# nianticlabs/simplerecon

Hardware: AMD Instinct MI355X
Metric: depth frames/sec (640x480, 7 src views, 64 planes) (higher is better)
Workload: dtype f32

## Files before the change

### simplerecon_amd/csrc/sr_pw_tiled.hip

```cpp
#include <stdlib.h>

#include "sr_common.h"

namespace {

typedef float pt_f16 __attribute__((ext_vector_type(16)));
typedef float pt_f4 __attribute__((ext_vector_type(4)));

constexpr int PT_KS = 32;
constexpr int PT_AROW = PT_KS + 4;

struct SrPtParams {
  const float* in; int in_sp;
  const float* wp;
  const float* bias; const float* gate;
  const float* res; int res_sp;
  float* out; int out_sp;
  int64_t part_stride;
  int M, HW, Cin, Cout, Co_pad, G;
  int slabs, slabs_per_part, ksplit, tiles_n;
  float slope;
};

template <int WM, int WN, int NTW, bool GATE>
__global__ __launch_bounds__(256, 2) void sr_pw_tiled_kernel(SrPtParams p) {
  constexpr int BM = 32 * WM, BN = 32 * WN * NTW;
  constexpr int A_FLOATS = BM * PT_AROW, B_FLOATS = (PT_KS / 8) * 2 * BN * 4;
  constexpr int A_PER_THREAD = BM * (PT_KS / 4) / 256;
  constexpr int B_PER_THREAD = (PT_KS / 8) * 2 * BN / 256;
  static_assert(WM * WN == 4 && A_PER_THREAD >= 1 && B_PER_THREAD >= 1, "4 waves; whole float4s per thread");
  extern __shared__ __attribute__((aligned(16))) float lds[];
  const int tid = threadIdx.x, lane = tid & 63, wave = __builtin_amdgcn_readfirstlane(tid >> 6);
  const int i = lane & 31, kk = lane >> 5;
  const int wm = wave / WN, wn = wave % WN;
  const int tile_n = blockIdx.x % p.tiles_n, tile_m = blockIdx.x / p.tiles_n;
  const int kpart = blockIdx.y;
  const int m0 = tile_m * BM, n0 = tile_n * BN;
  const int s_begin = kpart * p.slabs_per_part, s_end = min(p.slabs, s_begin + p.slabs_per_part);

  int a_row[A_PER_THREAD];
  const float* a_ptr[A_PER_THREAD];
  const float* g_ptr[A_PER_THREAD];
  const int a_q = tid & 7;
#pragma unroll
  for (int u = 0; u < A_PER_THREAD; ++u) {
    a_row[u] = (tid >> 3) + 32 * u;
    const int m = m0 + a_row[u];
    const bool ok = m < p.M;
    a_ptr[u] = ok ? p.in + (int64_t)m * p.in_sp + 4 * a_q : nullptr;
    g_ptr[u] = (GATE && ok) ? p.gate + (int64_t)(m / p.HW) * p.Cin + 4 * a_q : nullptr;
  }
  auto stage_load = [&](int s, pt_f4 (&ra)[A_PER_THREAD], pt_f4 (&rb)[B_PER_THREAD]) {
    const int k0 = s * PT_KS;
#pragma unroll
    for (int u = 0; u < A_PER_THREAD; ++u) {
      pt_f4 v = {0.f, 0.f, 0.f, 0.f};
      if (a_ptr[u] && k0 + 4 * a_q < p.Cin) {
        v = *reinterpret_cast<const pt_f4*>(a_ptr[u] + k0);
        if (GATE) v = v * *reinterpret_cast<const pt_f4*>(g_ptr[u] + k0);
      }
      ra[u] = v;
    }
#pragma unroll
    for (int u = 0; u < B_PER_THREAD; ++u) {
      const int e = tid + 256 * u;
      const int gh = e / BN, col = e - gh * BN;
      const int g = s * (PT_KS / 8) + (gh >> 1);
      pt_f4 v = {0.f, 0.f, 0.f, 0.f};
      if (g < p.G && n0 + col < p.Co_pad)
        v = *reinterpret_cast<const pt_f4*>(p.wp + ((int64_t)(g * 2 + (gh & 1)) * p.Co_pad + n0 + col) * 4);
      rb[u] = v;
    }
  };
  auto stage_store = [&](int buf, const pt_f4 (&ra)[A_PER_THREAD], const pt_f4 (&rb)[B_PER_THREAD]) {
    float* A = lds + buf * (A_FLOATS + B_FLOATS);
    float* Bt = A + A_FLOATS;
#pragma unroll
    for (int u = 0; u < A_PER_THREAD; ++u) *reinterpret_cast<pt_f4*>(&A[a_row[u] * PT_AROW + 4 * a_q]) = ra[u];
#pragma unroll
    for (int u = 0; u < B_PER_THREAD; ++u) *reinterpret_cast<pt_f4*>(&Bt[(tid + 256 * u) * 4]) = rb[u];
  };

  pt_f16 acc[NTW];
#pragma unroll
  for (int n = 0; n < NTW; ++n)
#pragma unroll
    for (int r = 0; r < 16; ++r) acc[n][r] = 0.0f;

  pt_f4 ra[A_PER_THREAD], rb[B_PER_THREAD];
  if (s_begin < s_end) {
    stage_load(s_begin, ra, rb);
    stage_store(0, ra, rb);
  }
  __syncthreads();
  for (int s = s_begin; s < s_end; ++s) {
    const int buf = (s - s_begin) & 1;
    const bool more = s + 1 < s_end;
    if (more) stage_load(s + 1, ra, rb);
    const float* A = lds + buf * (A_FLOATS + B_FLOATS);
    const float* Bt = A + A_FLOATS;
    const float* a_base = A + (32 * wm + i) * PT_AROW + 4 * kk;
    const float* b_base = Bt + (kk * BN + 32 * wn * NTW + i) * 4;
#pragma unroll
    for (int gl = 0; gl < PT_KS / 8; ++gl) {
      const pt_f4 a = *reinterpret_cast<const pt_f4*>(a_base + 8 * gl);
      pt_f4 b[NTW];
#pragma unroll
      for (int n = 0; n < NTW; ++n) b[n] = *reinterpret_cast<const pt_f4*>(b_base + (gl * 2 * BN + 32 * n) * 4);
#pragma unroll
      for (int e = 0; e < 4; ++e)
#pragma unroll
        for (int n = 0; n < NTW; ++n) acc[n] = __builtin_amdgcn_mfma_f32_32x32x2f32(a[e], b[n][e], acc[n], 0, 0, 0);
    }
    if (more) stage_store(buf ^ 1, ra, rb);
    __syncthreads();
  }

  const bool partial = p.ksplit > 1;
  const float slope = sr_uniform(partial ? -1.0f : p.slope);
  float* outp = p.out + (partial ? (int64_t)kpart * p.part_stride : (int64_t)0);
  const int rbase = m0 + 32 * wm + 4 * kk;
#pragma unroll
  for (int n = 0; n < NTW; ++n) {
    const int col = n0 + 32 * (wn * NTW + n) + i;
    const bool okc = col < p.Cout;
    const float bv = (!partial && p.bias && okc) ? p.bias[col] : 0.0f;
    float v[16];
#pragma unroll
    for (int r = 0; r < 16; ++r) v[r] = acc[n][r] + bv;
    if (!partial && p.res) {
      float rv[16];
#pragma unroll
      for (int r = 0; r < 16; ++r) {
        const int m = rbase + (r & 3) + 8 * (r >> 2);
        rv[r] = (okc && m < p.M) ? p.res[(int64_t)m * p.res_sp + col] : 0.0f;
      }
#pragma unroll
      for (int r = 0; r < 16; ++r) v[r] += rv[r];
    }
    sr_activate_group(v, slope);
#pragma unroll
    for (int r = 0; r < 16; ++r) {
      const int m = rbase + (r & 3) + 8 * (r >> 2);
      if (okc && m < p.M) outp[(int64_t)m * p.out_sp + col] = v[r];
    }
  }
}

int pt_num_cus() { return sr_device_cus(); }

struct PtPlan { int cfg, ks; };
constexpr int PT_BM[4] = {64, 128, 128, 64}, PT_BN[4] = {128, 160, 64, 64};

PtPlan pt_plan(int M, int Cin, int Cout, bool can_split) {
  const int f_cfg = sr_opt(SR_OPT_PT_CFG), f_ks = sr_opt(SR_OPT_PT_KS);
  const int slabs = (Cin + PT_KS - 1) / PT_KS;
  const long want = (long)pt_num_cus() * 3 / 2;
  PtPlan best = {0, 1};
  double best_cost = -1.0;
  for (int cfg = 0; cfg < 4; ++cfg) {
    if (f_cfg >= 0 && cfg != f_cfg) continue;
    const long tm = (M + PT_BM[cfg] - 1) / PT_BM[cfg], tn = (Cout + PT_BN[cfg] - 1) / PT_BN[cfg];
    const double pad = (double)(tm * PT_BM[cfg]) * (double)(tn * PT_BN[cfg]) / ((double)M * Cout);
    for (int ks = 1; ks <= 8; ks *= 2) {
      if (f_ks > 0 && ks != f_ks) continue;
      if (ks > 1 && (!can_split || slabs / ks < 4)) continue;
      const long wgs = tm * tn * ks;
      const double fill = wgs >= want ? 1.0 : (double)want / (double)wgs;
      const double reuse = 1.0 + 24.0 / (PT_BM[cfg] * PT_BN[cfg] / (double)(PT_BM[cfg] + PT_BN[cfg]));
      const double cost = pad * fill * reuse * (1.0 + (ks > 1 ? 0.10 + 2.0 * ks / slabs : 0.0));
      if (best_cost < 0 || cost < best_cost) { best = {cfg, ks}; best_cost = cost; }
    }
  }
  return best;
}

template <int WM, int WN, int NTW>
int pt_launch(const SrPtParams& p, int tiles_m, hipStream_t stream) {
  constexpr int BM = 32 * WM, BN = 32 * WN * NTW;
  const size_t lds = (size_t)2 * (BM * PT_AROW + (PT_KS / 8) * 2 * BN * 4) * sizeof(float);
  const dim3 grid((unsigned)(tiles_m * p.tiles_n), (unsigned)p.ksplit);
  if (p.gate) {
    hipError_t e = hipFuncSetAttribute((const void*)sr_pw_tiled_kernel<WM, WN, NTW, true>,
                                       hipFuncAttributeMaxDynamicSharedMemorySize, (int)lds);
    if (e != hipSuccess) return sr_hip_rc(e);
    hipLaunchKernelGGL((sr_pw_tiled_kernel<WM, WN, NTW, true>), grid, dim3(256), lds, stream, p);
  } else {
    hipError_t e = hipFuncSetAttribute((const void*)sr_pw_tiled_kernel<WM, WN, NTW, false>,
                                       hipFuncAttributeMaxDynamicSharedMemorySize, (int)lds);
    if (e != hipSuccess) return sr_hip_rc(e);
    hipLaunchKernelGGL((sr_pw_tiled_kernel<WM, WN, NTW, false>), grid, dim3(256), lds, stream, p);
  }
  return sr_hip_rc(hipGetLastError());
}

}

extern "C" size_t sr_pw_conv_tiled_workspace_bytes(int M, int Cin, int Cout) {
  if (M <= 0 || Cin <= 0 || Cout <= 0 || Cout % 4 != 0) return 0;
  const PtPlan pl = pt_plan(M, Cin, Cout, true);
  return pl.ks > 1 ? (size_t)pl.ks * M * Cout * sizeof(float) : 0;
}

extern "C" int sr_pw_conv_tiled_plan(int M, int Cin, int Cout, int can_split, int* cfg, int* ks) {
  if (M <= 0 || Cin <= 0 || Cout <= 0) return SR_ERR_INVALID_ARGUMENT;
  const PtPlan pl = pt_plan(M, Cin, Cout, can_split != 0 && Cout % 4 == 0);
  if (cfg) *cfg = pl.cfg;
  if (ks) *ks = pl.ks;
  return SR_OK;
}

extern "C" int sr_pw_conv_tiled_nhwc_fwd(const float* in, int in_pix_stride, const float* packed_w, const float* bias,
                                         const float* gate, const float* residual, int res_pix_stride, float* out,
                                         int out_pix_stride, int M, int HW, int Cin, int Cout, float act_code,
                                         void* workspace, size_t workspace_bytes, void* stream_) {
  if (M < 0 || HW <= 0 || Cin <= 0 || Cout <= 0) return SR_ERR_INVALID_ARGUMENT;
  if (M == 0) return SR_OK;
  if (!in || !packed_w || !out) return SR_ERR_INVALID_ARGUMENT;
  if (Cin % 4 != 0 || in_pix_stride % 4 != 0 || (((uintptr_t)in) & 15) != 0 || (gate && (((uintptr_t)gate) & 15) != 0))
    return SR_ERR_UNSUPPORTED;
  const bool can_split = workspace && (((uintptr_t)workspace) & 15) == 0 && Cout % 4 == 0 &&
                         (!residual || ((((uintptr_t)residual) & 15) == 0 && res_pix_stride % 4 == 0)) &&
                         (((uintptr_t)out) & 15) == 0 && out_pix_stride % 4 == 0 && (!bias || (((uintptr_t)bias) & 15) == 0);
  PtPlan pl = pt_plan(M, Cin, Cout, can_split);
  if (pl.ks > 1 && workspace_bytes < (size_t)pl.ks * M * Cout * sizeof(float)) pl = pt_plan(M, Cin, Cout, false);
  SrPtParams p;
  p.in = in; p.in_sp = in_pix_stride; p.wp = packed_w; p.bias = bias; p.gate = gate;
  p.res = residual; p.res_sp = res_pix_stride;
  p.M = M; p.HW = HW; p.Cin = Cin; p.Cout = Cout;
  p.Co_pad = ((Cout + 31) / 32) * 32;
  p.G = ((Cin + 63) / 64) * 8;
  p.slabs = (Cin + PT_KS - 1) / PT_KS;
  p.ksplit = pl.ks;
  p.slabs_per_part = (p.slabs + pl.ks - 1) / pl.ks;
  p.slope = act_code;
  p.part_stride = (int64_t)M * Cout;
  if (pl.ks > 1) { p.out = (float*)workspace; p.out_sp = Cout; }
  else { p.out = out; p.out_sp = out_pix_stride; }
  const int tiles_m = (M + PT_BM[pl.cfg] - 1) / PT_BM[pl.cfg];
  p.tiles_n = (Cout + PT_BN[pl.cfg] - 1) / PT_BN[pl.cfg];
  hipStream_t stream = (hipStream_t)stream_;
  int rc;
  switch (pl.cfg) {
    case 0: rc = pt_launch<2, 2, 2>(p, tiles_m, stream); break;
    case 1: rc = pt_launch<4, 1, 5>(p, tiles_m, stream); break;
    case 2: rc = pt_launch<4, 1, 2>(p, tiles_m, stream); break;
    default: rc = pt_launch<2, 2, 1>(p, tiles_m, stream); break;
  }
  if (rc == SR_OK && pl.ks > 1)
    rc = sr_launch_splitk_reduce((const float*)workspace, pl.ks, p.part_stride, bias, residual, (int64_t)0, res_pix_stride,
                                 out, (int64_t)0, out_pix_stride, 1, M, Cout, act_code, stream);
  return rc;
}
```

Measured before the change: 312.4.

## Stream pointwise GEMM tiles into LDS via buffer_load ... lds DMA with swizzle

For the non-gated pointwise tiled GEMM, global-to-LDS staging of the A activations and packed B weights now uses buffer_load_dwordx4 with the LDS-direct flag. This bypasses the register round trip and the separate LDS store. The A tile drops its padding and uses an XOR swizzle on the float4 column to avoid bank conflicts on the reads. Out-of-range rows and channels are masked through buffer OOB offsets. The risks are correctness of the swizzle and OOB handling, the inline asm juggling m0, and a full vmcnt(0) wait per stage, which may serialize the DMA against compute.

```diff
diff --git a/simplerecon_amd/csrc/sr_lds_dma.h b/simplerecon_amd/csrc/sr_lds_dma.h
--- /dev/null
+++ b/simplerecon_amd/csrc/sr_lds_dma.h
@@ -0,0 +1,40 @@
+#pragma once
+#include <stdint.h>
+
+#include <hip/hip_runtime.h>
+
+typedef unsigned int sr_dma_rsrc __attribute__((ext_vector_type(4)));
+constexpr unsigned SR_DMA_OOB = 0x7fffffffu;
+
+__device__ __forceinline__ sr_dma_rsrc sr_dma_make_rsrc(const void* base, unsigned bytes) {
+  const uint64_t a = (uint64_t)(uintptr_t)base;
+  sr_dma_rsrc r;
+  r[0] = __builtin_amdgcn_readfirstlane((unsigned)a);
+  r[1] = __builtin_amdgcn_readfirstlane((unsigned)(a >> 32) & 0xffffu);
+  r[2] = __builtin_amdgcn_readfirstlane(bytes);
+  r[3] = 0x00020000u;
+  return r;
+}
+
+__device__ __forceinline__ unsigned sr_lds_addr(const void* shared_ptr) {
+  return __builtin_amdgcn_readfirstlane((unsigned)(uintptr_t)shared_ptr);
+}
+
+__device__ __forceinline__ void sr_dma16(sr_dma_rsrc rsrc, unsigned voff, unsigned soff, unsigned lds_block) {
+  unsigned keep;
+  asm volatile(
+      "s_mov_b32 %0, m0\n\t"
+      "s_mov_b32 m0, %4\n\t"
+      "s_nop 0\n\t"
+      "buffer_load_dwordx4 %1, %2, %3 offen lds\n\t"
+      "s_mov_b32 m0, %0"
+      : "=&s"(keep)
+      : "v"(voff), "s"(rsrc), "s"(soff), "s"(lds_block)
+      : "memory");
+}
+
+template <int N>
+__device__ __forceinline__ void sr_dma_wait() {
+  static_assert(N >= 0 && N < 64, "vmcnt is a 6-bit counter");
+  asm volatile("s_waitcnt vmcnt(%0)" ::"n"(N) : "memory");
+}
diff --git a/simplerecon_amd/csrc/sr_pw_tiled.hip b/simplerecon_amd/csrc/sr_pw_tiled.hip
--- a/simplerecon_amd/csrc/sr_pw_tiled.hip
+++ b/simplerecon_amd/csrc/sr_pw_tiled.hip
@@ -1,6 +1,7 @@
 #include <stdlib.h>
 
 #include "sr_common.h"
+#include "sr_lds_dma.h"
 
 namespace {
 
@@ -29,6 +30,12 @@
   constexpr int A_PER_THREAD = BM * (PT_KS / 4) / 256;
   constexpr int B_PER_THREAD = (PT_KS / 8) * 2 * BN / 256;
   static_assert(WM * WN == 4 && A_PER_THREAD >= 1 && B_PER_THREAD >= 1, "4 waves; whole float4s per thread");
+#ifdef SR_PT_NO_DMA
+  constexpr bool DMA = false;
+#else
+  constexpr bool DMA = !GATE;
+#endif
+  constexpr int AROW = DMA ? PT_KS : PT_AROW;
   extern __shared__ __attribute__((aligned(16))) float lds[];
   const int tid = threadIdx.x, lane = tid & 63, wave = __builtin_amdgcn_readfirstlane(tid >> 6);
   const int i = lane & 31, kk = lane >> 5;
@@ -81,6 +88,34 @@
     for (int u = 0; u < B_PER_THREAD; ++u) *reinterpret_cast<pt_f4*>(&Bt[(tid + 256 * u) * 4]) = rb[u];
   };
 
+  const int d_rows = min(BM, p.M - m0);
+  const sr_dma_rsrc rs_a = sr_dma_make_rsrc(p.in + (int64_t)m0 * p.in_sp, (unsigned)((d_rows - 1) * p.in_sp + p.Cin) * 4u);
+  const sr_dma_rsrc rs_b = sr_dma_make_rsrc(p.wp, (unsigned)(p.G * 2 * p.Co_pad) * 16u);
+  const unsigned lds0 = sr_lds_addr(lds) + (unsigned)wave * 1024u;
+  const int d_q = (tid & 7) ^ ((tid >> 4) & 7);
+  unsigned d_aoff[A_PER_THREAD], d_boff[B_PER_THREAD];
+#pragma unroll
+  for (int u = 0; u < A_PER_THREAD; ++u)
+    d_aoff[u] = a_row[u] < d_rows ? (unsigned)(a_row[u] * p.in_sp + 4 * d_q) * 4u : SR_DMA_OOB;
+#pragma unroll
+  for (int u = 0; u < B_PER_THREAD; ++u) {
+    const int e = tid + 256 * u;
+    const int gh = e / BN, col = e - gh * BN;
+    d_boff[u] = n0 + col < p.Co_pad ? (unsigned)(gh * p.Co_pad + n0 + col) * 16u : SR_DMA_OOB;
+  }
+  auto stage_dma = [&](int s, int buf) {
+    const unsigned A = lds0 + (unsigned)(buf * (A_FLOATS + B_FLOATS)) * 4u, Bt = A + A_FLOATS * 4u;
+    const int k0 = s * PT_KS;
+    const bool chan_ok = k0 + 4 * d_q < p.Cin;
+    const bool grp_ok = s * (PT_KS / 8) + (PT_KS / 8) <= p.G;
+#pragma unroll
+    for (int u = 0; u < A_PER_THREAD; ++u)
+      sr_dma16(rs_a, chan_ok ? d_aoff[u] : SR_DMA_OOB, (unsigned)k0 * 4u, A + 4096u * u);
+#pragma unroll
+    for (int u = 0; u < B_PER_THREAD; ++u)
+      sr_dma16(rs_b, grp_ok ? d_boff[u] : SR_DMA_OOB, (unsigned)(s * (PT_KS / 8) * 2 * p.Co_pad) * 16u, Bt + 4096u * u);
+  };
+
   pt_f16 acc[NTW];
 #pragma unroll
   for (int n = 0; n < NTW; ++n)
@@ -89,21 +124,31 @@
 
   pt_f4 ra[A_PER_THREAD], rb[B_PER_THREAD];
   if (s_begin < s_end) {
-    stage_load(s_begin, ra, rb);
-    stage_store(0, ra, rb);
+    if (DMA) {
+      stage_dma(s_begin, 0);
+      sr_dma_wait<0>();
+    } else {
+      stage_load(s_begin, ra, rb);
+      stage_store(0, ra, rb);
+    }
   }
   __syncthreads();
+  const int a_sw = ((32 * wm + i) >> 1) & 7;
+  const int a_x = DMA ? (kk ^ a_sw) : kk;
   for (int s = s_begin; s < s_end; ++s) {
     const int buf = (s - s_begin) & 1;
     const bool more = s + 1 < s_end;
-    if (more) stage_load(s + 1, ra, rb);
+    if (more) {
+      if (DMA) stage_dma(s + 1, buf ^ 1);
+      else stage_load(s + 1, ra, rb);
+    }
     const float* A = lds + buf * (A_FLOATS + B_FLOATS);
     const float* Bt = A + A_FLOATS;
-    const float* a_base = A + (32 * wm + i) * PT_AROW + 4 * kk;
+    const float* a_base = A + (32 * wm + i) * AROW;
     const float* b_base = Bt + (kk * BN + 32 * wn * NTW + i) * 4;
 #pragma unroll
     for (int gl = 0; gl < PT_KS / 8; ++gl) {
-      const pt_f4 a = *reinterpret_cast<const pt_f4*>(a_base + 8 * gl);
+      const pt_f4 a = *reinterpret_cast<const pt_f4*>(a_base + (DMA ? 4 * (a_x ^ (2 * gl)) : 4 * a_x + 8 * gl));
       pt_f4 b[NTW];
 #pragma unroll
       for (int n = 0; n < NTW; ++n) b[n] = *reinterpret_cast<const pt_f4*>(b_base + (gl * 2 * BN + 32 * n) * 4);
@@ -112,7 +157,8 @@
 #pragma unroll
         for (int n = 0; n < NTW; ++n) acc[n] = __builtin_amdgcn_mfma_f32_32x32x2f32(a[e], b[n][e], acc[n], 0, 0, 0);
     }
-    if (more) stage_store(buf ^ 1, ra, rb);
+    if (DMA) sr_dma_wait<0>();
+    else if (more) stage_store(buf ^ 1, ra, rb);
     __syncthreads();
   }
 
```

Result: no change. 312.5 (median of 3 runs) (+0.0%).
